# biiiipy/JaxMARL-HFT

Hardware: AMD Instinct MI355X
Metric: env steps/sec (whole node), 2-agent MARL, 10-level LOB, NUM_ENVS=4096 (higher is better)
Workload: dtype int32

## Files before the change

### jaxmarl-hft_amd/csrc/hftlob.hip

```cpp
#include <hip/hip_runtime.h>
#include <stdint.h>
#include <string.h>
#include <stdio.h>
#include <mutex>
#include <type_traits>
#include <limits.h>

#include "../../include/hftlob.h"
#include "hftlob_draw.h"
#include "hftlob_internal.h"
#define HFTLOB_BAKED_QUAL static
#include "baked_cfgs.inc"

typedef int32_t i32;
typedef uint32_t u32;
typedef uint8_t u8;
#define DEV __device__ __forceinline__

DEV int lane_id() { return __lane_id(); }
DEV i32 rdl(i32 v, int l) { return __builtin_amdgcn_readlane(v, l); }
DEV i32 wrl(i32 old, i32 val, int l) { return __lane_id() == l ? val : old; }
DEV i32 uni(i32 v) { return __builtin_amdgcn_readfirstlane(v); }
DEV float unif(float v) { return __int_as_float(__builtin_amdgcn_readfirstlane(__float_as_int(v))); }
DEV i32 wadd(i32 a, i32 b) { return (i32)((u32)a + (u32)b); }
// ... 229 lines not shown
template <int S> DEV void ldcol(const i32* t, int R, int f, i32 (&o)[S]) {
    const int l = lane_id();
#pragma unroll
    for (int r = 0; r < S; ++r) o[r] = t[f * R + r * 64 + l];
}
DEV i32 ldu(const i32* t, int R, int f, int e) { return uni(t[f * R + e]); }
DEV void ld_msg(const i32* g, int4& x, int4& y) {
    x = reinterpret_cast<const int4*>(g)[0];
    y = reinterpret_cast<const int4*>(g)[1];
}
DEV void stu(i32* t, i32* scr, int R, int f, int e, i32 v) {
    const int l = lane_id();
    *(l == 0 ? t + f * R + e : scr + l) = v;
    lds_order();
}
DEV void st6(i32* t, i32* scr, int R, int e, i32 f0, i32 f1, i32 f2, i32 f3, i32 f4, i32 f5) {
    const int l = lane_id();
    i32 v = f0;
    v = wlane(v, f1, 1); v = wlane(v, f2, 2); v = wlane(v, f3, 3); v = wlane(v, f4, 4); v = wlane(v, f5, 5);
    *(l < 6 ? t + l * R + e : scr + l) = v;
    lds_order();
}
DEV void clr6(i32* t, i32* scr, int R, int e) {
    const int l = lane_id();
    *(l < 6 ? t + l * R + e : scr + l) = -1;
    lds_order();
}
DEV u32 ff1(lmask m) {
    u32 r;
    asm("s_ff1_i32_b64 %0, %1" : "=s"(r) : "s"(m));
    return r;
}
template <int S> DEV int first_slot(const lmask (&m)[S], int fallback) {
    u32 idx = ff1(m[0]);
#pragma unroll
    for (int r = 1; r < S; ++r) idx = min(idx, ff1(m[r]) | (u32)(64 * r));
    return idx == 0xFFFFFFFFu ? fallback : (int)idx;
}
template <int S> DEV int first_true(const bool (&pr)[S], int fallback) {
    lmask m[S];
#pragma unroll
    for (int r = 0; r < S; ++r) m[r] = bal(pr[r]);
    return first_slot(m, fallback);
}
template <int S> DEV i32 sget(const i32 (&a)[S], int e) {
    i32 v = a[0];
#pragma unroll
    for (int k = 1; k < S; ++k) v = (e >> 6) == k ? a[k] : v;
    return rdl(v, e & 63);
}

template <int S>
struct Side {
    i32* t;
    i32* scr;
    i32 best_p, best_q;
    i32 xp;
    i32 pc[S];
    i32 top, top_p, top_ts, top_tns;
    i32 rp, rq;
    lmask rm;
#ifdef HFTLOB_STAMPS_CHUNK
    u32 n_resc, n_rec;
#endif
};
template <bool LZ = false, int S> DEV void side_rec(Side<S>& s, u32 k) {
    s.rp = wlane(s.rp, s.best_p, (int)k);
    if (!LZ) s.rq = wlane(s.rq, s.best_q, (int)k);
    asm volatile("s_bitset1_b64 %0, %1" : "+s"(s.rm) : "s"(k));
#ifdef HFTLOB_STAMPS_CHUNK
    ++s.n_rec;
#endif
}

template <int S> DEV void col_set(i32 (&c)[S], int e, i32 v) {
    const int l = lane_id();
#pragma unroll
    for (int r = 0; r < S; ++r) c[r] = (l + 64 * r == e) ? v : c[r];
}

enum : u32 { F_STALE_A = 2, F_STALE_B = 4, F_CLEAN_A = 8, F_CLEAN_B = 16, F_NEG1_A = 32, F_NEG1_B = 64,
             F_PM1_A = 256, F_PM1_B = 512, F_LAZY = 0x20000000u, F_STALE_ANY = 0x40000000u, F_SLOW = 0x80000000u };
constexpr u32 STALE_ANY = F_STALE_ANY;
template <bool ASKS> struct SideBits {
    static constexpr u32 STALE = ASKS ? F_STALE_A : F_STALE_B;
    static constexpr u32 MARK = STALE | STALE_ANY;
    static constexpr u32 CLEAN = ASKS ? F_CLEAN_A : F_CLEAN_B;
    static constexpr u32 NEG1 = ASKS ? F_NEG1_A : F_NEG1_B;
    static constexpr u32 PM1 = ASKS ? F_PM1_A : F_PM1_B;
};
DEV u32 slow_bit(u32 fl) {
    return (fl & (F_CLEAN_A | F_CLEAN_B | F_NEG1_A | F_NEG1_B | F_PM1_A | F_PM1_B)) == (F_CLEAN_A | F_CLEAN_B)
               ? 0u : F_SLOW;
}

template <int S>
struct SideRows {
    int2 x0[S], x1[S], x2[S];
};
template <int S> DEV void fetch_side(SideRows<S>& f, const i32* g, const Valid<S>& V) {
    const int l = lane_id();
#pragma unroll
    for (int r = 0; r < S; ++r) {
        f.x0[r] = f.x1[r] = f.x2[r] = make_int2(-1, -1);
        if (V.v[r]) {
            const int2* row = reinterpret_cast<const int2*>(g + (r * 64 + l) * 6);
            f.x0[r] = row[0]; f.x1[r] = row[1]; f.x2[r] = row[2];
        }
    }
}
template <bool ASKS, int S>
DEV u32 commit_side(Side<S>& s, const SideRows<S>& f, int R, const Valid<S>& V) {
    const int l = lane_id();
    lmask bad = 0, n1 = 0, pm1 = 0;
#pragma unroll
    for (int r = 0; r < S; ++r) {
        const int sl = r * 64 + l;
        const i32 p = f.x0[r].x, q = f.x0[r].y, oid = f.x1[r].x, tid = f.x1[r].y, ts = f.x2[r].x, tns = f.x2[r].y;
        if (V.v[r]) {
            i32* t = s.t + sl;
            t[FP * R] = p; t[FQ * R] = q; t[FOID * R] = oid; t[FTID * R] = tid; t[FTS * R] = ts; t[FTNS * R] = tns;
        }
        s.pc[r] = V.v[r] ? p : -1;
        const u32 np_ = ~(u32)p, nq = ~(u32)q, no = ~(u32)oid, nt = ~(u32)tid, ns = ~(u32)ts, nn = ~(u32)tns;
        const u32 any0 = min(min(min(np_, nq), min(no, nt)), min(ns, nn));
        const u32 all0 = max(max(max(np_, nq), max(no, nt)), max(ns, nn));
        bad |= V.m[r] & bal((q <= 0) & (all0 != 0u));
        n1 |= V.m[r] & bal((p != -1) & (any0 == 0u));
        pm1 |= V.m[r] & bal((p == -1) & (all0 != 0u));
    }
    lds_order();
    s.top = -1;
    return (bad == 0ull ? SideBits<ASKS>::CLEAN : 0u) | (n1 != 0ull ? SideBits<ASKS>::NEG1 : 0u) |
           (pm1 != 0ull ? SideBits<ASKS>::PM1 : 0u);
}
template <int S> DEV void relink_side(Side<S>& s, int R, const Valid<S>& V) {
    i32 p[S];
    ldcol(s.t, R, FP, p);
#pragma unroll
    for (int r = 0; r < S; ++r) s.pc[r] = V.v[r] ? p[r] : -1;
    s.top = -1;
}
template <bool ASKS, int S> DEV u32 load_side(Side<S>& s, const i32* g, int R, const Valid<S>& V) {
    SideRows<S> f;
    fetch_side(f, g, V);
    return commit_side<ASKS>(s, f, R, V);
}
template <int S> DEV void store_side(const Side<S>& s, i32* g, int R, const Valid<S>& V) {
    const int l = lane_id();
#pragma unroll
    for (int r = 0; r < S; ++r) {
        const int sl = r * 64 + l;
        if (V.v[r]) {
            const i32* t = s.t + sl;
            int2* row = reinterpret_cast<int2*>(g + sl * 6);
            row[0] = make_int2(t[FP * R], t[FQ * R]);
            row[1] = make_int2(t[FOID * R], t[FTID * R]);
            row[2] = make_int2(t[FTS * R], t[FTNS * R]);
        }
    }
}
template <int S> DEV void clear_masked(Side<S>& s, int R, const lmask (&m)[S]) {
    const int l = lane_id();
#pragma unroll
    for (int r = 0; r < S; ++r) {
        const bool hit = (m[r] >> l) & 1ull;
// ... 97 lines not shown
    mtn_out = mtn;
    lmask pm[S];
#pragma unroll
    for (int r = 0; r < S; ++r) pm[r] = V.m[r] & bal(n[r] == mtn);
    return first_slot(pm, c.nO - 1);
}

struct Trades {
    i32* t;
    i32* scr;
    int R;
    DEV i32 get(int k, int r) const { return t[k * R + r * 64 + lane_id()]; }
    DEV i32 at(int k, int row) const { return uni(t[k * R + row]); }
};
template <int S> DEV void trades_fill(Trades& T, const Valid<S>& V, i32 v) {
    const int l = lane_id();
#pragma unroll
    for (int r = 0; r < S; ++r)
        if (V.v[r]) {
#pragma unroll
            for (int k = 0; k < 8; ++k) T.t[k * T.R + r * 64 + l] = v;
        }
    lds_order();
}
template <int S> DEV void load_trades(Trades& T, const i32* g, const Valid<S>& V) {
    const int l = lane_id();
#pragma unroll
    for (int r = 0; r < S; ++r) {
        if (V.v[r]) {
            const int o = r * 64 + l, R = T.R;
            const int4* row = reinterpret_cast<const int4*>(g + o * 8);
            const int4 a = row[0], b = row[1];
            T.t[0 * R + o] = a.x; T.t[1 * R + o] = a.y; T.t[2 * R + o] = a.z; T.t[3 * R + o] = a.w;
            T.t[4 * R + o] = b.x; T.t[5 * R + o] = b.y; T.t[6 * R + o] = b.z; T.t[7 * R + o] = b.w;
        }
    }
    lds_order();
}
template <int S> DEV void store_trades(const Trades& T, i32* g, const Valid<S>& V) {
    const int l = lane_id();
#pragma unroll
    for (int r = 0; r < S; ++r) {
        if (V.v[r]) {
            const int o = r * 64 + l, R = T.R;
            int4* row = reinterpret_cast<int4*>(g + o * 8);
            row[0] = make_int4(T.t[0 * R + o], T.t[1 * R + o], T.t[2 * R + o], T.t[3 * R + o]);
            row[1] = make_int4(T.t[4 * R + o], T.t[5 * R + o], T.t[6 * R + o], T.t[7 * R + o]);
        }
    }
}
DEV void trade_put(Trades& T, int e, i32 f0, i32 f1, i32 f2, i32 f3, i32 f4, i32 f5, i32 f6, i32 f7) {
    const int l = lane_id();
    i32 v = f0;
    v = wlane(v, f1, 1); v = wlane(v, f2, 2); v = wlane(v, f3, 3);
    v = wlane(v, f4, 4); v = wlane(v, f5, 5); v = wlane(v, f6, 6); v = wlane(v, f7, 7);
    *(l < 8 ? T.t + l * T.R + e : T.scr + l) = v;
    lds_order();
}

#ifndef HFTLOB_FILT_LOG2
#define HFTLOB_FILT_LOG2 12
#endif
constexpr int FILT_LOG2 = HFTLOB_FILT_LOG2, FILT_WORDS = 1 << (FILT_LOG2 - 5);
constexpr int PAD_FILT = 128, PAD_SCR = PAD_FILT + FILT_WORDS, PAD_WORDS = PAD_SCR + 64;
constexpr int PAD_CARRY = 96;
static_assert(FILT_WORDS >= 64 && FILT_WORDS % 64 == 0 && PAD_WORDS - PAD_SCR == 64, "filter words per lane, 64-word scratch row");
static_assert(PAD_CARRY + 13 <= PAD_FILT, "the rollout's 13 carry words end before the filter words");
__host__ __device__ constexpr int book_words(int nO, int nT) { return 12 * nO + 8 * nT + PAD_WORDS; }
template <int S>
struct Book {
    Side<S> a, b;
    Trades tr;
    Valid<S> vs, vt;
    LobCfg c;
    u32 fl;
    Key ek;
    i32 mi, nmsg;
    i32 ntr;
    bool part;
    i32* filt;
    bool filt_ok;
};

enum { H_ASK = 0, H_BID = 1, H_CNL_ASK = 2, H_CNL_BID = 3, H_NOP = 4, H_KIND = 7, H_DISCARD = 8, H_NEG1 = 16,
       H_PM1 = 32, H_MKT = 64, H_RARE = 128, H_MISS = 256, H_NOID = 512 };
struct Msg {
    i32 h, side, price, qty, oid, tid, t, tns;
    u32 k;
};

template <int S> DEV void top_new(Side<S>& s, int e, i32 np, i32 t, i32 tns, i32 maxint) {
    s.top = ((t != maxint) & (tns != maxint)) ? e : -1;
    s.top_p = np; s.top_ts = t; s.top_tns = tns;
}
template <int S> DEV void top_eq(Side<S>& s, int e, i32 t, i32 tns, i32 maxint) {
    if (fresh(t) > s.top_ts) return;
    asm volatile("");
    if (s.top < 0) return;
    asm volatile("");
    bool earlier = t < s.top_ts;
    if (!earlier) earlier = (tns < s.top_tns) | ((tns == s.top_tns) & (e < s.top));
    if (earlier) {
        s.top = tns != maxint ? e : -1;
        s.top_ts = t; s.top_tns = tns;
    }
}
#define XP_SET(s, v) ((s).xp = (v))
template <bool BID, int S, bool STALE_OK = true, bool NN = false, bool LZ = false>
DEV void note_add(Side<S>& s, u32& fl, int e, i32 np, i32 nq, i32 t, i32 tns, i32 maxint, u32 k) {
    constexpr u32 STALE = SideBits<!BID>::STALE, MARK = SideBits<!BID>::MARK;
    if (STALE_OK && (fl & STALE)) { s.top = -1; return; }
    const i32 bp = s.best_p;
    if (BID) {
        if (np < bp) {
            if (!NN && bp == -1) fl |= MARK;
        } else if (np > bp) {
            s.best_p = np;
            if (!LZ) s.best_q = nq;
            side_rec<LZ>(s, k);
            top_new(s, e, np, t, tns, maxint);
        } else if (!NN && bp == -1) {
            fl |= MARK;
        } else {
            if (!LZ) { s.best_q = wadd(s.best_q, nq); side_rec(s, k); }
            top_eq(s, e, t, tns, maxint);
        }
    } else if (NN && !STALE_OK) {
        const i32 xp = s.xp;
        if (np > xp) {
        } else if (np < xp) {
            s.best_p = np; if (!LZ) s.best_q = nq; XP_SET(s, np); side_rec<LZ>(s, k); top_new(s, e, np, t, tns, maxint);
        } else if (np == maxint) {
            fl |= MARK;
        } else {
            if (!LZ) { s.best_q = wadd(s.best_q, nq); side_rec(s, k); }
            top_eq(s, e, t, tns, maxint);
        }
    } else {
        if (np > bp) {
            if (bp == -1) {
                if (np == maxint) fl |= MARK;
                else { s.best_p = np; if (!LZ) s.best_q = nq; XP_SET(s, np); side_rec<LZ>(s, k); top_new(s, e, np, t, tns, maxint); }
            }
        } else if (np < bp) {
            if (NN || np != -1) { s.best_p = np; if (!LZ) s.best_q = nq; XP_SET(s, np); side_rec<LZ>(s, k); top_new(s, e, np, t, tns, maxint); }
        } else if (!NN && np == -1) {
            fl |= MARK;
        } else if (np != maxint) {
            if (!LZ) { s.best_q = wadd(s.best_q, nq); side_rec(s, k); }
            top_eq(s, e, t, tns, maxint);
        }
    }
}
template <bool ASKS, bool LZ = false, bool G = false, int S>
DEV void note_reduce(Side<S>& s, u32& fl, i32 op, i32 dq, u32 k, bool cleared) {
    constexpr u32 STALE = SideBits<ASKS>::STALE, MARK = SideBits<ASKS>::MARK;
    if (fl & STALE) return;
    if (op == s.best_p) {
        if (op == -1) {
            fl |= MARK;
        } else if (LZ) {
            if (G) {
                fl |= MARK;
            } else if (cleared) {
                lmask at = 0;
#pragma unroll
                for (int r = 0; r < S; ++r) at |= bal(s.pc[r] == op);
                if (at == 0ull) fl |= MARK;
// ... 39 lines not shown
    const i32 newq = imax_(0, wsub(qt, qtm));
    const i32 rem = wsub(qtm, qt);
    int e;
    if (B.ntr >= 0) {
        e = imin_(B.ntr, B.c.nT - 1);
        if (m.t != -1) B.ntr = imin_(B.ntr + 1, B.c.nT);
    } else {
        i32 tr4[S];
        ldcol(B.tr.t, B.tr.R, 4, tr4);
        lmask fm[S];
#pragma unroll
        for (int r = 0; r < S; ++r) fm[r] = B.vt.m[r] & bal(tr4[r] == -1);
        e = first_slot(fm, B.c.nT - 1);
    }
    trade_put(B.tr, e, pt, wmul(wsub(0, m.side), wsub(qt, newq)), ot, m.oid, m.t, m.tns, tt, m.tid);
    if (!G || (B.fl & SideBits<ASKS>::CLEAN)) {
        if (newq <= 0) side_clr(s, R, top);
        else stu(s.t, s.scr, R, FQ, top, newq);
        note_reduce<ASKS, LZ, G>(s, B.fl, pt, wsub(qt, newq), m.k, newq <= 0);
    } else {
        stu(s.t, s.scr, R, FQ, top, newq);
        rzn<ASKS>(s, B.fl, R, B.vs);
    }
    return rem;
}

template <bool BID, bool G, int S, bool POS = false, bool LZ = false>
DEV i32 match_against(Book<S>& B, Side<S>& s, i32 qtm, i32 price, const Msg& m) {
    const int R = B.c.nO;
    if (!POS && fresh(qtm) <= 0) return qtm;
    {
        const i32 bp = s.best_p;
        const i32 mp0 = (!BID && bp == -1) ? B.c.maxint : bp;
        if (__builtin_expect(BID ? mp0 < price : mp0 > price, 1)) return qtm;
    }
    while (qtm > 0) {
        if (B.fl & SideBits<!BID>::STALE) rescan<!BID, true, LZ>(s, B.fl, R, B.vs, B.c.maxint, m.k);
        i32 mp = s.best_p;
        if (!BID) {
            if (mp == -1) {
                if (price != B.c.maxint) break;
                mp = B.c.maxint;
            } else if (mp > price) {
                break;
            }
        } else if (mp < price) {
            break;
        }
        int top;
        i32 qt, ot, tt, tp;
        if (s.top >= 0 && s.top_p == mp) {
            top = s.top;
            qt = ldu(s.t, R, FQ, top); ot = ldu(s.t, R, FOID, top); tt = ldu(s.t, R, FTID, top);
            tp = mp;
        } else {
            i32 q[S], o[S], t[S], ts[S], tn[S], mts, mtn;
            ldcol(s.t, R, FTS, ts); ldcol(s.t, R, FTNS, tn);
            ldcol(s.t, R, FQ, q); ldcol(s.t, R, FOID, o); ldcol(s.t, R, FTID, t);
            top = top_idx(s.pc, ts, tn, B.vs, B.c, mp, mts, mtn);
            qt = sget(q, top); ot = sget(o, top); tt = sget(t, top); tp = sget(s.pc, top);
            s.top_p = mp; s.top_ts = mts; s.top_tns = mtn;
            s.top = ((tp == mp) & (mp != -1) & (mp != B.c.maxint) & (mts != B.c.maxint) & (mtn != B.c.maxint))
                        ? top : -1;
        }
        if (fresh(tp) == -1) break;
        asm volatile("");
        if (BID ? tp < price : tp > price) break;
        qtm = match_order<G, !BID, LZ>(B, s, top, qtm, m, qt, tp, ot, tt);
    }
    return qtm;
}

template <bool BID, bool G, bool LZ = false, int S>
DEV void add_order(Book<S>& B, Side<S>& s, const Msg& m, i32 qty, const lmask (&free)[S]) {
    const int R = B.c.nO;
    constexpr u32 CLEAN = SideBits<!BID>::CLEAN, NEG1 = SideBits<!BID>::NEG1, MARK = SideBits<!BID>::MARK,
                  PM1 = SideBits<!BID>::PM1;
    const i32 nq = imax_(0, qty);
    if (!G) {
        const int e = first_slot(free, R - 1);
        const bool was_empty = !no_slot(free);
        if (nq > 0) {
            side_put(s, R, e, m.price, nq, m.oid, m.tid, m.t, m.tns);
            if (m.h & (H_NEG1 | H_PM1)) B.fl = B.fl | (m.h & H_NEG1 ? NEG1 : 0u) | (m.h & H_PM1 ? PM1 : 0u) | F_SLOW;
            if (was_empty) note_add<BID, S, true, false, LZ>(s, B.fl, e, m.price, nq, m.t, m.tns, B.c.maxint, m.k);
            else { B.fl |= MARK; s.top = -1; }
        } else if (!was_empty) {
            side_clr(s, R, e);
            B.fl |= MARK;
        }
        return;
    }
    lmask fm[S];
    i32 q[S];
    ldcol(s.t, R, FQ, q);
    if ((B.fl & (CLEAN | NEG1 | PM1)) == CLEAN) {
#pragma unroll
        for (int r = 0; r < S; ++r) fm[r] = free[r];
    } else {
        i32 o[S], t[S], ts[S], tn[S];
        ldcol(s.t, R, FOID, o); ldcol(s.t, R, FTID, t);
        ldcol(s.t, R, FTS, ts); ldcol(s.t, R, FTNS, tn);
#pragma unroll
        for (int r = 0; r < S; ++r)
            fm[r] = B.vs.m[r] & (bal(s.pc[r] == -1) | bal(q[r] == -1) | bal(o[r] == -1) | bal(t[r] == -1) |
                                 bal(ts[r] == -1) | bal(tn[r] == -1));
    }
    const int e = first_slot(fm, R - 1);
    if (!(B.fl & CLEAN)) {
        side_put(s, R, e, m.price, nq, m.oid, m.tid, m.t, m.tns);
        if (m.h & H_PM1) B.fl |= PM1;
        rzn<!BID>(s, B.fl, R, B.vs);
        return;
    }
    const i32 op = sget(s.pc, e), oq = sget(q, e);
    const bool was_empty = (op == -1) & (oq == -1);
    if (nq > 0) {
        side_put(s, R, e, m.price, nq, m.oid, m.tid, m.t, m.tns);
        if (m.h & H_NEG1) B.fl |= NEG1;
        if (m.h & H_PM1) B.fl |= PM1;
        if (was_empty) note_add<BID, S, true, false, LZ>(s, B.fl, e, m.price, nq, m.t, m.tns, B.c.maxint, m.k);
        else { B.fl |= MARK; s.top = -1; }
    } else if (!was_empty) {
        side_clr(s, R, e);
        B.fl |= MARK;
    }
}

template <bool BID, int S> DEV void evict_if_full(Book<S>& B, Side<S>& s, lmask (&free)[S]) {
    const int R = B.c.nO;
    lmask neg = 0;
#pragma unroll
    for (int r = 0; r < S; ++r) neg |= B.vs.m[r] & bal(s.pc[r] < 0);
    if (neg != 0ull) return;
    i32 w = BID ? INT_MAX : INT_MIN;
#pragma unroll
    for (int r = 0; r < S; ++r)
        w = BID ? imin_(w, B.vs.v[r] ? s.pc[r] : INT_MAX) : imax_(w, B.vs.v[r] ? s.pc[r] : INT_MIN);
    const i32 worst = BID ? wave_min(w) : wave_max(w);
    lmask m[S];
#pragma unroll
    for (int r = 0; r < S; ++r) m[r] = B.vs.m[r] & bal(s.pc[r] == worst);
    const i32 top = s.top;
    clear_masked(s, R, m);
    s.top = worst != s.top_p ? top : -1;
    if ((worst == s.best_p) | (s.best_p == -1)) B.fl |= SideBits<!BID>::MARK;
#pragma unroll
    for (int r = 0; r < S; ++r) free[r] = m[r];
}
template <bool BID, bool RARE, int S, bool POS = false, bool LZ = false>
DEV void add_free(Book<S>& B, Side<S>& s, const Msg& m, i32 qty, const lmask (&free)[S]) {
    const int R = B.c.nO;
    if (!POS && qty <= 0) return;
    u32 e;
    if (S == 2) {
        if (free[0] != 0ull) {
            e = ff1(free[0]);
            s.pc[0] = wlane(s.pc[0], m.price, (int)e);
        } else {
            e = ff1(free[S - 1]);
            s.pc[S - 1] = wlane(s.pc[S - 1], m.price, (int)e);
            e |= 64u;
        }
        st6(s.t, s.scr, R, (int)e, m.price, qty, m.oid, m.tid, m.t, m.tns);
    } else {
        e = ff1(free[0]);
#pragma unroll
        for (int r = 1; r < S; ++r) e = min(e, ff1(free[r]) | (u32)(64 * r));
        side_put(s, R, (int)e, m.price, qty, m.oid, m.tid, m.t, m.tns);
    }
    if (RARE && __builtin_expect((m.h & (H_NEG1 | H_PM1)) != 0, 0)) {
        asm volatile("");
        constexpr u32 NEG1 = SideBits<!BID>::NEG1, PM1 = SideBits<!BID>::PM1;
        B.fl = B.fl | (m.h & H_NEG1 ? NEG1 : 0u) | (m.h & H_PM1 ? PM1 : 0u) | F_SLOW;
    }
    note_add<BID, S, false, !RARE, LZ>(s, B.fl, (int)e, m.price, qty, m.t, m.tns, B.c.maxint, m.k);
}
template <bool BID, bool LZ = false, int S> DEV bool add_common(Book<S>& B, Side<S>& s, const Msg& m, const lmask (&free)[S]) {
#ifndef HFTLOB_OLD_ADD_TEST
    if (S == 2) {
        if (__builtin_expect(free[0] != 0ull, 1)) {
            add_free<BID, false, S, true, LZ>(B, s, m, m.qty, free);
            return true;
        }
        if (free[S - 1] == 0ull) return false;
        add_free<BID, false, S, true, LZ>(B, s, m, m.qty, free);
        return true;
    }
#endif
    if (no_slot(free)) return false;
    add_free<BID, false, S, true, LZ>(B, s, m, m.qty, free);
    return true;
}
template <bool G, bool RARE, bool LZ = false, int S> DEV void bid_lim(Book<S>& B, Msg m) {
    if (!RARE) __builtin_assume(m.qty > 0);
    constexpr bool POS = !RARE && !G;
    if (POS) {
        if (__builtin_expect(B.a.xp > m.price, 1)) {
            lmask free[S];
            free_slots(B, B.b, free);
            if (add_common<true, LZ>(B, B.b, m, free)) return;
            if (B.c.check_fill) evict_if_full<true>(B, B.b, free);
            add_order<true, G, LZ>(B, B.b, m, m.qty, free);
            return;
        }
    }
    const i32 rem = match_against<false, G, S, POS, LZ>(B, B.a, m.qty, m.price, m);
    if (RARE && __builtin_expect((m.h & H_MKT) != 0, 0)) m.price = B.c.maxint;
    lmask free[S];
    free_slots(B, B.b, free);
    if (!no_slot(free)) {
        if (!G) add_free<true, RARE, S, false, LZ>(B, B.b, m, (RARE && (m.h & H_DISCARD)) ? 0 : rem, free);
        else if (!(m.h & H_DISCARD)) add_order<true, G, LZ>(B, B.b, m, rem, free);
        return;
    }
    if (B.c.check_fill) evict_if_full<true>(B, B.b, free);
    if (!(m.h & H_DISCARD)) add_order<true, G, LZ>(B, B.b, m, rem, free);
}
template <bool G, bool RARE, bool LZ = false, int S> DEV void ask_lim(Book<S>& B, Msg m) {
    if (!RARE) __builtin_assume(m.qty > 0);
    if (RARE && __builtin_expect((m.h & H_MKT) != 0, 0)) m.price = 0;
    constexpr bool POS = !RARE && !G;
    if (POS && __builtin_expect(B.b.best_p < m.price, 1)) {
        lmask free[S];
        free_slots(B, B.a, free);
        if (add_common<false, LZ>(B, B.a, m, free)) return;
        if (B.c.check_fill) evict_if_full<false>(B, B.a, free);
        add_order<false, G, LZ>(B, B.a, m, m.qty, free);
        return;
    }
    const i32 rem = match_against<true, G, S, POS, LZ>(B, B.b, m.qty, m.price, m);
    lmask free[S];
    free_slots(B, B.a, free);
    if (!no_slot(free)) {
        if (!G) add_free<false, RARE, S, false, LZ>(B, B.a, m, (RARE && (m.h & H_DISCARD)) ? 0 : rem, free);
        else if (!(m.h & H_DISCARD)) add_order<false, G, LZ>(B, B.a, m, rem, free);
        return;
    }
    if (B.c.check_fill) evict_if_full<false>(B, B.a, free);
    if (!(m.h & H_DISCARD)) add_order<false, G, LZ>(B, B.a, m, rem, free);
}
template <int S>
DEV int random_id_match(const Book<S>& B, Key& k, const i32 (&o)[S], const lmask (&pm)[S]) {
    k = split_key(k, 2, 0, B.part);
    lmask w[S];
    int tot = 0;
#pragma unroll
    for (int r = 0; r < S; ++r) {
        w[r] = pm[r] & bal(o[r] != 0);
        tot += __builtin_popcountll(w[r]);
    }
    const u32 bits = random_bits(k, 1, 0, B.part);
    const float u = __uint_as_float((bits >> 9) | 0x3f800000u) - 1.0f;
    const float rr = (float)tot * (1.0f - u);
    i32 chosen = 0;
    if (tot > 0) {
        int K = (int)ceilf(rr);
#pragma unroll
        for (int r = 0; r < S; ++r) {
            const int c = __builtin_popcountll(w[r]);
            if (K > 0 && K <= c) {
                const u32 below = __builtin_amdgcn_mbcnt_hi((u32)(w[r] >> 32), __builtin_amdgcn_mbcnt_lo((u32)w[r], 0u));
                const lmask hit = w[r] & bal(below == (u32)(K - 1));
                chosen = rdl(o[r], (int)ff1(hit));
            }
            K -= c;
        }
    }
    lmask f[S];
#pragma unroll
    for (int r = 0; r < S; ++r) f[r] = B.vs.m[r] & bal(o[r] == chosen);
    return first_slot(f, -1);
}
template <bool G, bool ASKS, bool RC, bool LZ = false, int S> DEV void cancel(Book<S>& B, Side<S>& s, const Msg& m) {
    if (!G && m.qty == 0) return;
    const int R = B.c.nO;
    int idx;
    i32 op, oq;
    if (!RC && (m.h & H_MISS)) {
        idx = R - 1;
        op = sget(s.pc, R - 1);
#ifndef HFTLOB_NO_MISS_EMPTY
        if (!G && fresh(op) == -1) return;
        asm volatile("");
#endif
        oq = ldu(s.t, R, FQ, R - 1);
    } else {
    i32 o[S], q[S];
    ldcol(s.t, R, FOID, o);
    ldcol(s.t, R, FQ, q);
    lmask fm[S];
    idx = -1;
    if (RC || !(m.h & H_NOID)) {
#pragma unroll
        for (int r = 0; r < S; ++r) fm[r] = B.vs.m[r] & bal(o[r] == m.oid);
        idx = first_slot(fm, -1);
    }
    if (idx < 0) {
        const i32 lo = wsub(B.c.init_id, wmul(B.c.depth, 2));
        const u32 span = (u32)wsub(B.c.init_id, lo);
        u32 d[S];
#pragma unroll
        for (int r = 0; r < S; ++r) d[r] = (u32)wsub(o[r], lo);
        vkeep_sets(d);
#pragma unroll
        for (int r = 0; r < S; ++r) d[r] = s.pc[r] == m.price ? d[r] : 0xFFFFFFFFu;
        vkeep_sets(d);
#pragma unroll
        for (int r = 0; r < S; ++r) d[r] = q[r] >= m.qty ? d[r] : 0xFFFFFFFFu;
        vkeep_sets(d);
#pragma unroll
        for (int r = 0; r < S; ++r) fm[r] = B.vs.m[r] & bal(d[r] <= span);
        if (!RC) {
            idx = first_slot(fm, R - 1);
        } else {
            idx = first_slot(fm, -1);
            if (idx < 0 && B.c.cancel_mode >= 2) {
                Key k = split_key(B.ek, B.nmsg, B.mi, B.part);
#pragma unroll
                for (int r = 0; r < S; ++r) fm[r] = B.vs.m[r] & bal(s.pc[r] == m.price) & bal(q[r] >= m.qty);
                idx = random_id_match(B, k, o, fm);
                if (idx < 0 && B.c.cancel_mode == 3) {
#pragma unroll
                    for (int r = 0; r < S; ++r) fm[r] = B.vs.m[r] & bal(s.pc[r] == m.price);
                    idx = random_id_match(B, k, o, fm);
                }
            }
            if (idx < 0) idx = R - 1;
        }
    }
    op = sget(s.pc, idx);
    oq = sget(q, idx);
    }
    if (!G && fresh(op & oq) == -1) {
        asm volatile("");
        if (m.qty >= -1) return;
#ifndef HFTLOB_NO_MISS_EMPTY
        B.fl |= SideBits<ASKS>::PM1 | F_SLOW;
#endif
    }
    const i32 nq = wsub(oq, m.qty);
    if (!G || (B.fl & SideBits<ASKS>::CLEAN)) {
        if (nq <= 0) side_clr(s, R, idx);
        else stu(s.t, s.scr, R, FQ, idx, nq);
        note_reduce<ASKS, LZ, G>(s, B.fl, op, wsub(oq, nq > 0 ? nq : 0), m.k, nq <= 0);
    } else {
        stu(s.t, s.scr, R, FQ, idx, nq);
        rzn<ASKS>(s, B.fl, R, B.vs);
    }
}

DEV void decode_msgs(const LobCfg& c, int4& x, const int4& y) {
    const i32 ty = x.x, sd = ty == 4 ? wsub(0, x.y) : x.y;
    const bool cnl = (ty == 2) | (ty == 3);
    i32 h = H_ASK;
    h = (((ty == 0) & (sd == 0))) ? H_NOP : h;
    h = (((ty == 1) | (ty == 4)) & (sd == 1)) ? H_BID : h;
    h = (cnl & (sd == 1)) ? H_CNL_BID : h;
    h = (cnl & (sd == -1)) ? H_CNL_ASK : h;
    if (((c.t4 == 0) | (c.t4 == 2)) & (ty == 4)) h |= H_DISCARD;
    const i32 p_add = c.t4 == 2 ? (h == H_BID ? c.maxint : 0) : x.w;
    if ((p_add != -1) & ((y.x == -1) | (y.y == -1) | (y.z == -1) | (y.w == -1))) h |= H_NEG1;
    if (p_add == -1) h |= H_PM1;
    if (c.t4 == 2) h |= H_MKT;
    if (h & (H_DISCARD | H_NEG1 | H_PM1 | H_MKT)) h |= H_RARE;
    if ((h <= H_BID) & (x.z <= 0)) h |= H_RARE;
    if (((h & H_KIND) == H_ASK) & (sd != -1)) h |= H_RARE;
    if ((h <= H_BID) & (x.w < 0)) h |= H_RARE;
    x.x = h;
    x.y = sd;
}
template <bool G, bool RC, bool LZ = false, int S>
DEV void process_msg_(Book<S>& B, u32 k, i32 h, i32 sdv, i32 d2, i32 d3, i32 d4, i32 d5, i32 d6, i32 d7) {
    Msg m;
    m.h = h; m.side = 0; m.price = d3; m.qty = d2; m.oid = d4; m.tid = d5; m.t = d6; m.tns = d7;
    m.k = k;
    const i32 kind = h & H_KIND;
    if (kind == H_CNL_ASK) cancel<G, true, RC, LZ>(B, B.a, m);
    else if (kind == H_CNL_BID) cancel<G, false, RC, LZ>(B, B.b, m);
    else if (kind == H_BID) {
        if (!G && !(h & H_RARE)) {
            m.side = 1;
            bid_lim<G, false, LZ>(B, m);
        } else {
            m.side = rdl(sdv, k);
            bid_lim<G, true, LZ>(B, m);
        }
    } else if (kind == H_ASK) {
        if (!G && !(h & H_RARE)) {
            m.side = -1;
            ask_lim<G, false, LZ>(B, m);
        } else {
            m.side = rdl(sdv, k);
            ask_lim<G, true, LZ>(B, m);
        }
    }
}

DEV i32 ffill(i32 v, i32 carry) {
    const int l = lane_id();
    const lmask m = bal(v != -1) & (~0ull >> (63 - l));
    const int src = m ? 63 - __builtin_clzll(m) : -1;
    const i32 got = __builtin_amdgcn_ds_bpermute(src << 2, v);
    return src < 0 ? carry : got;
}
template <bool REC = true, bool LZ = false, int S> DEV void refresh_best(Book<S>& B, u32 k = 0) {
    if (B.fl & STALE_ANY) {
        if (B.fl & F_STALE_A) rescan<true, REC, LZ>(B.a, B.fl, B.c.nO, B.vs, B.c.maxint, k);
        if (B.fl & F_STALE_B) rescan<false, REC, LZ>(B.b, B.fl, B.c.nO, B.vs, B.c.maxint, k);
        B.fl &= ~STALE_ANY;
    }
}

DEV u32 hash_id(i32 v) { return ((u32)v * 0x9E3779B1u) >> (32 - FILT_LOG2); }
DEV u32 hash_px(i32 p, bool ask) { return (((u32)p * 0x85EBCA6Bu) ^ (ask ? 0xC2B2AE35u : 0x27D4EB2Fu)) >> (32 - FILT_LOG2); }
DEV void filt_set(i32* f, u32 h, bool on) {
    __hip_atomic_fetch_or(reinterpret_cast<u32*>(f) + (h >> 5), on ? 1u << (h & 31) : 0u, __ATOMIC_RELAXED,
                          __HIP_MEMORY_SCOPE_WORKGROUP);
}
DEV u32 filt_get(const i32* f, u32 h) { return ((u32)f[h >> 5] >> (h & 31)) & 1u; }
DEV u32 lanes_below(lmask m) { return __builtin_amdgcn_mbcnt_hi((u32)(m >> 32), __builtin_amdgcn_mbcnt_lo((u32)m, 0u)); }
template <int S> DEV int side_room(const Book<S>& B, const Side<S>& s) {
    const int R = B.c.nO, rl = (R - 1) >> 6, ll = (R - 1) & 63;
    int n = 0;
    bool last = false;
#pragma unroll
    for (int r = 0; r < S; ++r) {
        lmask f = B.vs.m[r] & bal(s.pc[r] == -1);
        if (r == rl) {
            last = (f >> ll) & 1ull;
            f &= ~(1ull << ll);
        }
        n += __builtin_popcountll(f);
    }
    if (!last) return -1;
    return ldu(s.t, R, FQ, R - 1) == -1 ? n : -1;
}
template <bool RC, int S> DEV lmask chunk_noops(Book<S>& B, const int4& x, const int4& y, int cnt, i32& hf) {
    const int l = lane_id();
    const i32 kind = x.x & H_KIND, qty = x.z, price = x.w, oid = y.x;
    const bool in = l < cnt;
    const lmask nop = bal(in & (kind == H_NOP));
    hf = 0;
    if ((i32)B.fl < 0) {
        B.filt_ok = false;
        return nop;
    }
    const bool cnl = (kind == H_CNL_ASK) | (kind == H_CNL_BID), add = (kind == H_ASK) | (kind == H_BID);
    const i32 lo = wsub(B.c.init_id, wmul(B.c.depth, 2));
    const u32 span = (u32)wsub(B.c.init_id, lo);
    const bool init_oid = (u32)wsub(oid, lo) <= span;
    const lmask brk = bal(in & ((add & (((x.x & (H_NEG1 | H_PM1)) != 0) | init_oid)) | (cnl & (qty < -1))));
    const lmask before = brk ? (1ull << ff1(brk)) - 1ull : ~0ull;
    const lmask zero = bal(in & cnl & (qty == 0)) & before;
    if (RC || (u32)wsub(-1, lo) <= span) return nop | zero;
    i32* f = B.filt;
    if (!B.filt_ok) {
#pragma unroll
        for (int w = 0; w < FILT_WORDS; w += 64) f[w + l] = 0;
        wave_sync();
        const int R = B.c.nO;
#pragma unroll
        for (int sd = 0; sd < 2; ++sd) {
            const Side<S>& s = sd ? B.b : B.a;
            i32 o[S];
            ldcol(s.t, R, FOID, o);
#pragma unroll
            for (int r = 0; r < S; ++r) {
                filt_set(f, hash_id(o[r]), B.vs.v[r] & (o[r] != -1));
                filt_set(f, hash_px(s.pc[r], sd == 0), B.vs.v[r] & ((u32)wsub(o[r], lo) <= span));
            }
        }
    }
    filt_set(f, hash_id(oid), in & add);
    B.filt_ok = brk == 0ull;
    wave_sync();
    const bool ask = kind == H_CNL_ASK;
    const u32 hid = filt_get(f, hash_id(oid)), hpx = filt_get(f, hash_px(price, ask));
    const bool hit = (hid | hpx) != 0u;
    const int room_a = side_room(B, B.a), room_b = side_room(B, B.b);
    const u32 adds_a = lanes_below(bal(in & (kind == H_ASK))), adds_b = lanes_below(bal(in & (kind == H_BID)));
    const int room = ask ? room_a : room_b;
    const i32 adds = (i32)(ask ? adds_a : adds_b);
    const bool cmiss = in & cnl & (oid != -1) & !hit;
    const bool quiet = cmiss & (qty >= -1) & (room >= 0) & (adds <= room);
#ifndef HFTLOB_NO_MISS
    const bool cnd = in & cnl & (oid != -1) & (hid == 0u) & (((before >> l) & 1ull) != 0ull);
    hf = cnd ? (hpx == 0u ? (i32)H_MISS : (i32)H_NOID) : 0;
#endif
    return nop | zero | (bal(quiet) & before);
}

#ifdef HFTLOB_STAMPS_CHUNK
#define CHUNK_PARAMS , unsigned long long &acc_pre, unsigned long long &acc_loop
#define CHUNK_ARGS , acc_pre, acc_loop
#else
#define CHUNK_PARAMS
#define CHUNK_ARGS
#endif
template <bool RC, bool LZ = false, int S>
DEV void run_chunk(Book<S>& B, const int4& x, const int4& y, int cnt, int base, i32& rpa, i32& rqa, i32& rpb,
                   i32& rqb CHUNK_PARAMS) {
#ifdef HFTLOB_STAMPS_CHUNK
    const unsigned long long tp0 = __builtin_amdgcn_s_memtime();
#endif
    const lmask live = cnt >= 64 ? ~0ull : (1ull << cnt) - 1ull;
#ifdef HFTLOB_NO_SKIP
    const lmask skip = 0;
    const i32 hx = x.x;
#else
    i32 hf;
    const lmask skip = chunk_noops<RC>(B, x, y, cnt, hf) & live;
    const i32 hx = x.x | hf;
#endif
    lmask todo = live & ~skip;
#ifdef HFTLOB_KO_LOOP
    todo = 0;
#endif
    refresh_best<false, LZ>(B);
    const i32 cpa = B.a.best_p, cqa = LZ ? 0 : B.a.best_q, cpb = B.b.best_p, cqb = LZ ? 0 : B.b.best_q;
    B.a.rm = B.b.rm = 0ull;
    B.a.rp = B.b.rp = 0;
    if (!LZ) B.a.rq = B.b.rq = 0;
#ifdef HFTLOB_STAMPS_CHUNK
    const unsigned long long tp1 = __builtin_amdgcn_s_memtime();
    acc_pre += tp1 - tp0;
#endif
    if (todo) {
        u32 k = ff1(todo);
        i32 h = rdl(hx, k), d2 = rdl(x.z, k), d3 = rdl(x.w, k), d4 = rdl(y.x, k),
            d5 = rdl(y.y, k), d6 = rdl(y.z, k), d7 = rdl(y.w, k);
        do {
            asm volatile("s_bitset0_b64 %0, %1" : "+s"(todo) : "s"(k));
            if (RC) B.mi = base + (int)k;
            if ((i32)B.fl >= 0) process_msg_<false, RC, LZ>(B, k, h, x.y, d2, d3, d4, d5, d6, d7);
            else process_msg_<true, RC, LZ>(B, k, h, x.y, d2, d3, d4, d5, d6, d7);
            refresh_best<true, LZ>(B, k);
            const u32 kn = ff1(todo);
            h = rdl(hx, kn); d2 = rdl(x.z, kn); d3 = rdl(x.w, kn);
            d4 = rdl(y.x, kn); d5 = rdl(y.y, kn); d6 = rdl(y.z, kn); d7 = rdl(y.w, kn);
            k = kn;
        } while (todo);
    }
#ifdef HFTLOB_STAMPS_CHUNK
    acc_loop += __builtin_amdgcn_s_memtime() - tp1;
#endif
    {
        const int l = lane_id();
        const lmask below = ~0ull >> (63 - l);
        const lmask ma = B.a.rm & below, mb = B.b.rm & below;
        const int sa = ma ? 63 - __builtin_clzll(ma) : -1, sb = mb ? 63 - __builtin_clzll(mb) : -1;
        const i32 gpa = __builtin_amdgcn_ds_bpermute(sa << 2, B.a.rp), gqa = LZ ? 0 : __builtin_amdgcn_ds_bpermute(sa << 2, B.a.rq);
        const i32 gpb = __builtin_amdgcn_ds_bpermute(sb << 2, B.b.rp), gqb = LZ ? 0 : __builtin_amdgcn_ds_bpermute(sb << 2, B.b.rq);
        rpa = sa < 0 ? cpa : gpa;
        rqa = sa < 0 ? cqa : gqa;
        rpb = sb < 0 ? cpb : gpb;
        rqb = sb < 0 ? cqb : gqb;
    }
}

template <int S> DEV void book_bind(Book<S>& B, i32* lds) {
    B.a.t = lds;
    B.b.t = lds + 6 * B.c.nO;
    B.tr.t = lds + 12 * B.c.nO;
    B.tr.R = B.c.nT;
    B.filt = lds + 12 * B.c.nO + 8 * B.c.nT + PAD_FILT;
    B.filt_ok = false;
#ifdef HFTLOB_STAMPS_CHUNK
    B.a.n_resc = B.a.n_rec = B.b.n_resc = B.b.n_rec = 0;
#endif
    B.a.scr = B.b.scr = B.tr.scr = lds + 12 * B.c.nO + 8 * B.c.nT + PAD_SCR;
    B.vs.init(B.c.nO);
    B.vt.init(B.c.nT);
}

template <int S, bool RC>
__global__ __launch_bounds__(64) void k_book_process(hftlob_lob_cfg cfg, int n_env, int n_msg, const u32* __restrict__ keys,
                                                     const i32* __restrict__ msgs,
                                                     i32* __restrict__ asks, i32* __restrict__ bids,
                                                     i32* __restrict__ trades, i32* __restrict__ best_asks,
                                                     i32* __restrict__ best_bids) {
    one_wave();
    extern __shared__ __attribute__((aligned(16))) i32 lds[];
    const int e = blockIdx.x;
    if (e >= n_env) return;
    const int l = lane_id();
    Book<S> B;
    B.c = lobcfg(cfg);
    book_bind(B, lds);
    const int R = B.c.nO;
    i32* ga = asks + (size_t)e * R * 6;
    i32* gb = bids + (size_t)e * R * 6;
    i32* gt = trades + (size_t)e * B.c.nT * 8;
    B.fl = load_side<true>(B.a, ga, R, B.vs) | load_side<false>(B.b, gb, R, B.vs) | F_STALE_A | F_STALE_B | STALE_ANY;
    B.fl |= slow_bit(B.fl);
    load_trades(B.tr, gt, B.vt);
    {
        lmask fr[S], bad = 0;
#pragma unroll
        for (int r = 0; r < S; ++r) fr[r] = B.vt.m[r] & bal(B.tr.get(4, r) == -1);
        const int first = first_slot(fr, B.c.nT);
        const int l = lane_id();
#pragma unroll
        for (int r = 0; r < S; ++r) bad |= B.vt.m[r] & ~fr[r] & bal(r * 64 + l >= first);
        B.ntr = bad == 0ull ? first : -1;
    }
    if (RC) {
        B.ek = Key{keys[2 * e], keys[2 * e + 1]};
        B.nmsg = n_msg;
        B.part = cfg.prng_partitionable;
    }
    const i32* gm = msgs + (size_t)e * n_msg * 8;
    int4 nx = make_int4(0, 0, 0, 0), ny = nx;
    if (l < n_msg) {
        ld_msg(gm + l * 8, nx, ny);
    }
    for (int base = 0; base < n_msg; base += 64) {
        const int row = base + l;
        int4 x = nx, y = ny;
        nx = make_int4(0, 0, 0, 0);
// ... 1338 lines not shown

template <int S>
__global__ __launch_bounds__(64) void k_book_depth(hftlob_lob_cfg cfg, int n_env, int n_levels,
                                                   const i32* __restrict__ asks, const i32* __restrict__ bids,
                                                   i32* __restrict__ depth) {
    one_wave();
    extern __shared__ __attribute__((aligned(16))) i32 lds[];
    const int e = blockIdx.x;
    if (e >= n_env) return;
    const int l = lane_id();
    Book<S> B;
    B.c = lobcfg(cfg);
    book_bind(B, lds);
    const int R = B.c.nO;
    load_side<true>(B.a, asks + (size_t)e * R * 6, R, B.vs);
    load_side<false>(B.b, bids + (size_t)e * R * 6, R, B.vs);
    i32 v = 0;
    v = depth_side<false>(B.a, R, B.vs, B.c.maxint, n_levels, v);
    v = depth_side<true>(B.b, R, B.vs, B.c.maxint, n_levels, v);
    if (l < 4 * n_levels) depth[(size_t)e * 4 * n_levels + l] = v;
}

template <int S, bool RC>
__global__ __launch_bounds__(64) void k_book_process_depth(hftlob_lob_cfg cfg, int n_env, int n_msg,
                                                           const u32* __restrict__ keys, const i32* __restrict__ msgs,
                                                           i32* __restrict__ asks, i32* __restrict__ bids,
                                                           i32* __restrict__ trades, int n_levels, int n_keep,
                                                           i32* __restrict__ depth, i32* __restrict__ all_asks,
                                                           i32* __restrict__ all_bids) {
    one_wave();
    extern __shared__ __attribute__((aligned(16))) i32 lds[];
    const int e = blockIdx.x;
    if (e >= n_env) return;
    const int l = lane_id();
    Book<S> B;
    B.c = lobcfg(cfg);
    book_bind(B, lds);
    const int R = B.c.nO;
    i32* ga = asks + (size_t)e * R * 6;
    i32* gb = bids + (size_t)e * R * 6;
    i32* gt = trades + (size_t)e * B.c.nT * 8;
    B.fl = load_side<true>(B.a, ga, R, B.vs) | load_side<false>(B.b, gb, R, B.vs) | F_STALE_A | F_STALE_B | STALE_ANY;
    B.fl |= slow_bit(B.fl);
    load_trades(B.tr, gt, B.vt);
    {
        lmask fr[S], bad = 0;
#pragma unroll
        for (int r = 0; r < S; ++r) fr[r] = B.vt.m[r] & bal(B.tr.get(4, r) == -1);
        const int first = first_slot(fr, B.c.nT);
#pragma unroll
        for (int r = 0; r < S; ++r) bad |= B.vt.m[r] & ~fr[r] & bal(r * 64 + l >= first);
        B.ntr = bad == 0ull ? first : -1;
    }
    if (RC) {
        B.ek = Key{keys[2 * e], keys[2 * e + 1]};
        B.nmsg = n_msg;
        B.part = cfg.prng_partitionable;
    }
    const int first_kept = n_msg - n_keep;
    const int dw = 4 * n_levels;
    i32* gd = depth ? depth + (size_t)e * n_keep * dw : nullptr;
    i32* gsa = all_asks ? all_asks + (size_t)e * n_keep * R * 6 : nullptr;
    i32* gsb = all_asks ? all_bids + (size_t)e * n_keep * R * 6 : nullptr;
    i32 dv = 0;
    u32 dirty = 3u;
    const i32* gm = msgs + (size_t)e * n_msg * 8;
    int4 nx = make_int4(0, 0, 0, 0), ny = nx;
    if (l < n_msg) {
        ld_msg(gm + l * 8, nx, ny);
    }
    for (int base = 0; base < n_msg; base += 64) {
        const int row = base + l;
        int4 x = nx, y = ny;
        nx = make_int4(0, 0, 0, 0);
        ny = nx;
        if (row + 64 < n_msg) {
            ld_msg(gm + (row + 64) * 8, nx, ny);
        }
        decode_msgs(B.c, x, y);
        const int cnt = uni(imin_(64, n_msg - base));
        const lmask live = cnt >= 64 ? ~0ull : (1ull << cnt) - 1ull;
        i32 hf;
        const lmask skip = chunk_noops<RC>(B, x, y, cnt, hf) & live;
        const i32 hx = x.x | hf;
        refresh_best<false>(B);
        B.a.rm = B.b.rm = 0ull;
        B.a.rp = B.a.rq = B.b.rp = B.b.rq = 0;
        for (int k = 0; k < cnt; ++k) {
            if (!((skip >> k) & 1ull)) {
                const i32 h = rdl(hx, k), d2 = rdl(x.z, k), d3 = rdl(x.w, k), d4 = rdl(y.x, k), d5 = rdl(y.y, k),
                          d6 = rdl(y.z, k), d7 = rdl(y.w, k);
                const i32 ntr0 = B.ntr;
                if (RC) B.mi = base + k;
                if ((i32)B.fl >= 0) process_msg_<false, RC>(B, (u32)k, h, x.y, d2, d3, d4, d5, d6, d7);
                else process_msg_<true, RC>(B, (u32)k, h, x.y, d2, d3, d4, d5, d6, d7);
                refresh_best(B, (u32)k);
#ifdef HFTLOB_DEPTH_BOTH
                (void)ntr0;
                dirty = 3u;
#else
                const i32 kind = h & H_KIND;
                const bool add = kind <= H_BID;
                const bool no_trade = (ntr0 >= 0) & (ntr0 < B.c.nT) & (B.ntr == ntr0) & (d6 != -1);
                dirty |= ((kind == H_ASK) | (kind == H_CNL_ASK)) ? 1u : 2u;
                if (add & !no_trade) dirty = 3u;
#endif
            }
            const int j = base + k - first_kept;
            if (j >= 0) {
                if (gd) {
                    if (dirty & 1u) dv = depth_side<false>(B.a, R, B.vs, B.c.maxint, n_levels, dv);
                    if (dirty & 2u) dv = depth_side<true>(B.b, R, B.vs, B.c.maxint, n_levels, dv);
                    dirty = 0u;
                    if (l < dw) gd[(size_t)j * dw + l] = dv;
                }
                if (gsa) {
                    store_side(B.a, gsa + (size_t)j * R * 6, R, B.vs);
                    store_side(B.b, gsb + (size_t)j * R * 6, R, B.vs);
                }
            }
        }
    }
    store_side(B.a, ga, R, B.vs);
    store_side(B.b, gb, R, B.vs);
    store_trades(B.tr, gt, B.vt);
}

#define MAX_AGENT_ROWS 128

constexpr u32 INFO_F32_MM = 0xC0B9FFu, INFO_F32_EXE = 0x13Cu;
constexpr u32 TALLY_SUM_LANES = 0x34u;
struct TallyLane { double a, b; };
DEV int tally_word(int l) { return l < 25 ? 8 + 2 * l : (l < 40 ? l - 32 : 58 + 2 * (l - 40)); }
DEV TallyLane tally_load(const double* row, bool all) {
    const int l = lane_id();
    const bool hdr = (l >= 32) & (l < 40);
    TallyLane t{0.0, 0.0};
    if ((l < 25) | hdr | ((l >= 40) & all)) {
        const int w = tally_word(l);
        t.a = row[w];
        t.b = row[hdr ? (((TALLY_SUM_LANES >> (l - 32)) & 1u) ? 2 : 3) : w + 1];
    }
    return t;
}
DEV void tally_store(double* row, const TallyLane& t, float rew, const i32 (&iw)[HFTLOB_INFO_AGENT_WORDS], u32 f32,
                     bool all) {
    const int l = lane_id();
    const int k = l < 25 ? l - 1 : l - 40;
    i32 v = 0;
#pragma unroll
    for (int j = 0; j < HFTLOB_INFO_AGENT_WORDS; ++j) v = k == j ? iw[j] : v;
    double x = ((f32 >> (k & 31)) & 1u) ? (double)bitf(v) : (double)v;
    if (l == 0) x = (double)rew;
    if ((l >= 32) & (l < 40)) {
        const int h = l - 32;
        const double run = t.b + (((TALLY_SUM_LANES >> h) & 1u) ? (double)rew : 1.0);
        double a;
        if (h == 0) a = t.a + 1.0;
        else if (h == 1) a = t.a + (all ? 1.0 : 0.0);
        else if (h < 4) a = all ? 0.0 : run;
        else if ((h & 1) == 0) a = all ? t.a + run : t.a;
        else a = all ? t.a + run * run : t.a;
        row[h] = a;
    } else if ((l < 25) | ((l >= 40) & all)) {
        const int w = tally_word(l);
        row[w] = t.a + x;
        row[w + 1] = t.b + x * x;
    }
}
template <int S, int NFIX, bool RC, bool RA = false, bool QUIET = false, int PK = -1, bool TALLY = false,
          int BAKED = -1, bool DRAWN = false>
DEV bool env_step_dev(const hftlob_env_cfg& c_rt, int key_n, int ek, int e, const u32* __restrict__ keys, bool master,
                      Key& mk,
                      i32* __restrict__ actions_io, const i32* __restrict__ msg_data,
                      const i32* __restrict__ init_states, i32* __restrict__ state, float* __restrict__ obs_out,
                      float* __restrict__ rew_out, u8* __restrict__ done_all_out, u8* __restrict__ dones_out,
                      i32* __restrict__ info_out, i32* __restrict__ obs_raw_out, i32* __restrict__ msgs_out,
                      i32* __restrict__ debug_out, i32* lds, bool resident, bool keep, u32& fl_carry,
                      const i32* pre_keys = nullptr, bool emit_rt = true, double* __restrict__ stats = nullptr,
// ... 1584 lines not shown
```

Baseline: 104.8 million.

## Dispatch messages by precomputed class combining kind, rare and slow-mode bits

Re-encodes the per-message header so that kind, a rare flag and a general-path flag fit in a 5-bit class. The hot loop then dispatches with a single compare chain straight to the fast limit and cancel handlers. The general-path bit is recomputed for the whole chunk only when a rescan happens, and setting the slow flag now also marks the book stale so that recomputation fires. This is meant to cut branch and flag-check overhead per message, at the cost of extra bookkeeping and a more intricate header encoding.

```diff
diff --git a/jaxmarl-hft_amd/csrc/hftlob.hip b/jaxmarl-hft_amd/csrc/hftlob.hip
--- a/jaxmarl-hft_amd/csrc/hftlob.hip
+++ b/jaxmarl-hft_amd/csrc/hftlob.hip
@@ -335,6 +335,7 @@
 enum : u32 { F_STALE_A = 2, F_STALE_B = 4, F_CLEAN_A = 8, F_CLEAN_B = 16, F_NEG1_A = 32, F_NEG1_B = 64,
              F_PM1_A = 256, F_PM1_B = 512, F_LAZY = 0x20000000u, F_STALE_ANY = 0x40000000u, F_SLOW = 0x80000000u };
 constexpr u32 STALE_ANY = F_STALE_ANY;
+constexpr u32 GO_SLOW = F_SLOW | F_STALE_ANY;
 template <bool ASKS> struct SideBits {
     static constexpr u32 STALE = ASKS ? F_STALE_A : F_STALE_B;
     static constexpr u32 MARK = STALE | STALE_ANY;
@@ -598,8 +599,8 @@
     bool filt_ok;
 };
 
-enum { H_ASK = 0, H_BID = 1, H_CNL_ASK = 2, H_CNL_BID = 3, H_NOP = 4, H_KIND = 7, H_DISCARD = 8, H_NEG1 = 16,
-       H_PM1 = 32, H_MKT = 64, H_RARE = 128, H_MISS = 256, H_NOID = 512 };
+enum { H_ASK = 0, H_BID = 1, H_CNL_ASK = 2, H_CNL_BID = 3, H_NOP = 4, H_KIND = 7, H_RARE = 8, H_GEN = 16, H_CLASS = 31,
+       H_DISCARD = 32, H_NEG1 = 64, H_PM1 = 128, H_MKT = 256, H_MISS = 512, H_NOID = 1024 };
 struct Msg {
     i32 h, side, price, qty, oid, tid, t, tns;
     u32 k;
@@ -805,7 +806,7 @@
         const bool was_empty = !no_slot(free);
         if (nq > 0) {
             side_put(s, R, e, m.price, nq, m.oid, m.tid, m.t, m.tns);
-            if (m.h & (H_NEG1 | H_PM1)) B.fl = B.fl | (m.h & H_NEG1 ? NEG1 : 0u) | (m.h & H_PM1 ? PM1 : 0u) | F_SLOW;
+            if (m.h & (H_NEG1 | H_PM1)) B.fl = B.fl | (m.h & H_NEG1 ? NEG1 : 0u) | (m.h & H_PM1 ? PM1 : 0u) | GO_SLOW;
             if (was_empty) note_add<BID, S, true, false, LZ>(s, B.fl, e, m.price, nq, m.t, m.tns, B.c.maxint, m.k);
             else { B.fl |= MARK; s.top = -1; }
         } else if (!was_empty) {
@@ -895,7 +896,7 @@
     if (RARE && __builtin_expect((m.h & (H_NEG1 | H_PM1)) != 0, 0)) {
         asm volatile("");
         constexpr u32 NEG1 = SideBits<!BID>::NEG1, PM1 = SideBits<!BID>::PM1;
-        B.fl = B.fl | (m.h & H_NEG1 ? NEG1 : 0u) | (m.h & H_PM1 ? PM1 : 0u) | F_SLOW;
+        B.fl = B.fl | (m.h & H_NEG1 ? NEG1 : 0u) | (m.h & H_PM1 ? PM1 : 0u) | GO_SLOW;
     }
     note_add<BID, S, false, !RARE, LZ>(s, B.fl, (int)e, m.price, qty, m.t, m.tns, B.c.maxint, m.k);
 }
@@ -1059,7 +1060,7 @@
         asm volatile("");
         if (m.qty >= -1) return;
 #ifndef HFTLOB_NO_MISS_EMPTY
-        B.fl |= SideBits<ASKS>::PM1 | F_SLOW;
+        B.fl |= SideBits<ASKS>::PM1 | GO_SLOW;
 #endif
     }
     const i32 nq = wsub(oq, m.qty);
@@ -1086,19 +1087,29 @@
     if ((p_add != -1) & ((y.x == -1) | (y.y == -1) | (y.z == -1) | (y.w == -1))) h |= H_NEG1;
     if (p_add == -1) h |= H_PM1;
     if (c.t4 == 2) h |= H_MKT;
-    if (h & (H_DISCARD | H_NEG1 | H_PM1 | H_MKT)) h |= H_RARE;
-    if ((h <= H_BID) & (x.z <= 0)) h |= H_RARE;
-    if (((h & H_KIND) == H_ASK) & (sd != -1)) h |= H_RARE;
-    if ((h <= H_BID) & (x.w < 0)) h |= H_RARE;
+    const bool add = (h & H_KIND) <= H_BID;
+    bool rare = (h & (H_DISCARD | H_NEG1 | H_PM1 | H_MKT)) != 0;
+    rare |= x.z <= 0;
+    rare |= ((h & H_KIND) == H_ASK) & (sd != -1);
+    rare |= x.w < 0;
+    if (add & rare) h |= H_RARE;
     x.x = h;
     x.y = sd;
 }
+template <bool REC = true, bool LZ = false, int S> DEV u32 refresh_best(Book<S>& B, u32 k = 0) {
+    if (B.fl & STALE_ANY) {
+        if (B.fl & F_STALE_A) rescan<true, REC, LZ>(B.a, B.fl, B.c.nO, B.vs, B.c.maxint, k);
+        if (B.fl & F_STALE_B) rescan<false, REC, LZ>(B.b, B.fl, B.c.nO, B.vs, B.c.maxint, k);
+        B.fl &= ~STALE_ANY;
+        return true;
+    }
+    return false;
+}
+DEV i32 class_gen(u32 fl, i32 hx) { return (hx & ~(i32)H_GEN) | ((i32)fl < 0 ? (i32)H_GEN : 0); }
 template <bool G, bool RC, bool LZ = false, int S>
-DEV void process_msg_(Book<S>& B, u32 k, i32 h, i32 sdv, i32 d2, i32 d3, i32 d4, i32 d5, i32 d6, i32 d7) {
-    Msg m;
-    m.h = h; m.side = 0; m.price = d3; m.qty = d2; m.oid = d4; m.tid = d5; m.t = d6; m.tns = d7;
-    m.k = k;
-    const i32 kind = h & H_KIND;
+DEV void process_kind_(Book<S>& B, Msg& m, i32 sdv) {
+    const i32 h = m.h, kind = h & H_KIND;
+    const u32 k = m.k;
     if (kind == H_CNL_ASK) cancel<G, true, RC, LZ>(B, B.a, m);
     else if (kind == H_CNL_BID) cancel<G, false, RC, LZ>(B, B.b, m);
     else if (kind == H_BID) {
@@ -1119,6 +1130,44 @@
         }
     }
 }
+template <bool RC, bool LZ = false, int S> DEV void process_class_(Book<S>& B, Msg& m, i32 sdv) {
+    const i32 c = m.h & H_CLASS;
+    if (c == H_BID) { m.side = 1; bid_lim<false, false, LZ>(B, m); return; }
+    asm volatile("");
+    if (c == H_ASK) { m.side = -1; ask_lim<false, false, LZ>(B, m); return; }
+    asm volatile("");
+    if (c == H_CNL_ASK) { cancel<false, true, RC, LZ>(B, B.a, m); return; }
+    asm volatile("");
+    if (c == H_CNL_BID) { cancel<false, false, RC, LZ>(B, B.b, m); return; }
+    asm volatile("");
+    if (m.h & H_GEN) {
+        process_kind_<true, RC, LZ>(B, m, sdv);
+    } else {
+        const i32 kind = m.h & H_KIND;
+        m.side = rdl(sdv, m.k);
+        if (kind == H_BID) bid_lim<false, true, LZ>(B, m);
+        else if (kind == H_ASK) ask_lim<false, true, LZ>(B, m);
+    }
+}
+template <bool RC, bool LZ = false, bool CLS = true, int S>
+DEV void process_msg_(Book<S>& B, i32& hx, u32 k, i32 h, i32 sdv, i32 d2, i32 d3, i32 d4, i32 d5, i32 d6, i32 d7) {
+    Msg m;
+    m.h = h; m.side = 0; m.price = d3; m.qty = d2; m.oid = d4; m.tid = d5; m.t = d6; m.tns = d7;
+    m.k = k;
+#ifdef HFTLOB_OLD_DISPATCH
+    constexpr bool BY_CLASS = false;
+#else
+    constexpr bool BY_CLASS = CLS;
+#endif
+    if (BY_CLASS) {
+        process_class_<RC, LZ>(B, m, sdv);
+        if (refresh_best<true, LZ>(B, k)) hx = class_gen(B.fl, hx);
+    } else {
+        if ((i32)B.fl >= 0) process_kind_<false, RC, LZ>(B, m, sdv);
+        else process_kind_<true, RC, LZ>(B, m, sdv);
+        refresh_best<true, LZ>(B, k);
+    }
+}
 
 DEV i32 ffill(i32 v, i32 carry) {
     const int l = lane_id();
@@ -1127,14 +1176,6 @@
     const i32 got = __builtin_amdgcn_ds_bpermute(src << 2, v);
     return src < 0 ? carry : got;
 }
-template <bool REC = true, bool LZ = false, int S> DEV void refresh_best(Book<S>& B, u32 k = 0) {
-    if (B.fl & STALE_ANY) {
-        if (B.fl & F_STALE_A) rescan<true, REC, LZ>(B.a, B.fl, B.c.nO, B.vs, B.c.maxint, k);
-        if (B.fl & F_STALE_B) rescan<false, REC, LZ>(B.b, B.fl, B.c.nO, B.vs, B.c.maxint, k);
-        B.fl &= ~STALE_ANY;
-    }
-}
-
 DEV u32 hash_id(i32 v) { return ((u32)v * 0x9E3779B1u) >> (32 - FILT_LOG2); }
 DEV u32 hash_px(i32 p, bool ask) { return (((u32)p * 0x85EBCA6Bu) ^ (ask ? 0xC2B2AE35u : 0x27D4EB2Fu)) >> (32 - FILT_LOG2); }
 DEV void filt_set(i32* f, u32 h, bool on) {
@@ -1230,11 +1271,11 @@
     const lmask live = cnt >= 64 ? ~0ull : (1ull << cnt) - 1ull;
 #ifdef HFTLOB_NO_SKIP
     const lmask skip = 0;
-    const i32 hx = x.x;
+    i32 hx = class_gen(B.fl, x.x);
 #else
     i32 hf;
     const lmask skip = chunk_noops<RC>(B, x, y, cnt, hf) & live;
-    const i32 hx = x.x | hf;
+    i32 hx = class_gen(B.fl, x.x | hf);
 #endif
     lmask todo = live & ~skip;
 #ifdef HFTLOB_KO_LOOP
@@ -1256,9 +1297,7 @@
         do {
             asm volatile("s_bitset0_b64 %0, %1" : "+s"(todo) : "s"(k));
             if (RC) B.mi = base + (int)k;
-            if ((i32)B.fl >= 0) process_msg_<false, RC, LZ>(B, k, h, x.y, d2, d3, d4, d5, d6, d7);
-            else process_msg_<true, RC, LZ>(B, k, h, x.y, d2, d3, d4, d5, d6, d7);
-            refresh_best<true, LZ>(B, k);
+            process_msg_<RC, LZ>(B, hx, k, h, x.y, d2, d3, d4, d5, d6, d7);
             const u32 kn = ff1(todo);
             h = rdl(hx, kn); d2 = rdl(x.z, kn); d3 = rdl(x.w, kn);
             d4 = rdl(y.x, kn); d5 = rdl(y.y, kn); d6 = rdl(y.z, kn); d7 = rdl(y.w, kn);
@@ -2763,7 +2802,7 @@
         const lmask live = cnt >= 64 ? ~0ull : (1ull << cnt) - 1ull;
         i32 hf;
         const lmask skip = chunk_noops<RC>(B, x, y, cnt, hf) & live;
-        const i32 hx = x.x | hf;
+        i32 hx = x.x | hf;
         refresh_best<false>(B);
         B.a.rm = B.b.rm = 0ull;
         B.a.rp = B.a.rq = B.b.rp = B.b.rq = 0;
@@ -2773,9 +2812,7 @@
                           d6 = rdl(y.z, k), d7 = rdl(y.w, k);
                 const i32 ntr0 = B.ntr;
                 if (RC) B.mi = base + k;
-                if ((i32)B.fl >= 0) process_msg_<false, RC>(B, (u32)k, h, x.y, d2, d3, d4, d5, d6, d7);
-                else process_msg_<true, RC>(B, (u32)k, h, x.y, d2, d3, d4, d5, d6, d7);
-                refresh_best(B, (u32)k);
+                process_msg_<RC, false, false>(B, hx, (u32)k, h, x.y, d2, d3, d4, d5, d6, d7);
 #ifdef HFTLOB_DEPTH_BOTH
                 (void)ntr0;
                 dirty = 3u;
```

New measurement: 105.2 million, median of 6. Within noise of the previous version (+0.4%).
